# schwallergroup/matinvent

Hardware: AMD Instinct MI355X
Metric: crystal structures/sec (1000-step reverse diffusion) (higher is better)
Workload: dtype f32 via 2-plane fp16 split (3 fp16 MFMA terms, f32 accumulate)

## Files before the change

### matinvent_amd/csrc/edge_stage.hip

```cpp
#include <mutex>

#include <cstdio>
#include <cstdlib>
#include "net.h"
#include "gemm_split.h"
#define MI_LOOP_BARRIER() __builtin_amdgcn_s_barrier()
#define MI_RING_WAIT(w) asm volatile("s_waitcnt vmcnt(20)" : "+v"((w)[0][0]), "+v"((w)[0][1]), "+v"((w)[1][0]), "+v"((w)[1][1]))

namespace mi {

extern int g_edge2_train;
int g_edge2_fused = 1;

#if MI_PLANES_FP16

struct EdgeGemm2Args {
    Planes A;
    const u16* W2f;
    const float* b2;
    const float* dsc;
    const int* src;
    const int* rowptr;
    float* part;
    int E, N;
    const int* tab = nullptr;
    float* Z2 = nullptr;
    unsigned long long* clk;
};

constexpr int EG2_TAB = 2 + 128 + 128;
__global__ __launch_bounds__(128) void edge2_tables_kernel(const int* __restrict__ src, const int* __restrict__ rowptr, int E, int N, int* __restrict__ tab) {
    const int tile = blockIdx.x, tid = threadIdx.x, row0 = tile * 128;
    if (row0 >= E) return;
    const int nrows = E - row0 < 128 ? E - row0 : 128;
    const int node_first = src[row0];
    int* t = tab + (size_t)tile * EG2_TAB;
    const int r = row0 + tid, node = node_first + tid;
    t[2 + tid] = r < E ? src[r] - node_first : -1;
    t[130 + tid] = node < N ? tile - (rowptr[node] >> 7) : 0;
    if (tid == 0) {
        t[0] = node_first;
        t[1] = src[row0 + nrows - 1] - node_first + 1;
    }
}

constexpr int EG2B_STAGE = 2 * 128 * 64, EG2B_NST = 4;
constexpr int EG2B_LDS = EG2B_NST * EG2B_STAGE + 128 * 4 + 128 * 4;

template <int D, bool SAVE_Z = false>
__global__ __launch_bounds__(256) __attribute__((amdgpu_waves_per_eu(2, 2))) void edge_gemm2b_kernel(EdgeGemm2Args a) {
    constexpr int H = 512, KS = H / 16, KT = H / 32;
    extern __shared__ __attribute__((aligned(16))) unsigned char smem[];
    int* srcl = reinterpret_cast<int*>(smem + EG2B_NST * EG2B_STAGE);
    int* slotb = srcl + 128;
    const int tid = threadIdx.x, lane = tid & 63, wave = __builtin_amdgcn_readfirstlane(tid >> 6);
    const int l31 = lane & 31, kg = lane >> 5;
    const int id = blockIdx.x, slot = id >> 3, half = slot & 1, tile = (slot >> 1) * 8 + (id & 7);
    const int row0 = tile * 128;
    if (row0 >= a.E) return;
    const int nrows = a.E - row0 < 128 ? a.E - row0 : 128;
    int stamp_i = 0;
    auto stamp = [&]() {
        if (a.clk && tid == 0) a.clk[(size_t)(tile * 2 + half) * 8 + stamp_i] = __builtin_amdgcn_s_memtime();
        ++stamp_i;
    };
    stamp();
    if (a.clk && tid == 0) a.clk[(size_t)(tile * 2 + half) * 8 + 4] = __builtin_amdgcn_s_memrealtime();

    const int* tab = a.tab + (size_t)tile * EG2_TAB;
    int t_srcl = -1, t_slotb = 0;
    if (tid < 128) {
        t_srcl = tab[2 + tid];
        t_slotb = tab[130 + tid];
    }
    const int node_first = tab[0], cnt_tab = tab[1];

    const __amdgpu_buffer_rsrc_t rsa = uniform_rsrc(a.A.base + a.A.tile(tile, 0), a.A.KT * 24576);
    const int voffa = (lane >> 2) * 64 + (((lane & 3) ^ ((lane >> 4) & 3)) << 4);
    auto dma_tile = [&](int kt, int st) {
#pragma unroll
        for (int q = 0; q < 4; ++q) {
            const int piece = wave * 4 + q;
            __builtin_amdgcn_raw_ptr_buffer_load_lds(rsa, (__attribute__((address_space(3))) void*)(smem + st * EG2B_STAGE + piece * 1024), 16, voffa,
                                                     kt * 24576 + (piece >> 3) * 8192 + (piece & 7) * 1024, 0, 0);
        }
    };
    dma_tile(0, 0);
    dma_tile(1, 1);
    dma_tile(2, 2);

    int voffw[2];
#pragma unroll
    for (int t = 0; t < 2; ++t) voffw[t] = lane * 16 + ((8 * half + 2 * wave + t) * KS) * 2048;
    u32x4 ring[D][2][2];
    const u32x4 rsw_s = rsrc_words(a.W2f, H * H * 4);
    auto ring_load = [&](int ks, u32x4 (&w)[2][2]) {
        const int soff = __builtin_amdgcn_readfirstlane(ks * 2048);
#pragma unroll
        for (int t = 0; t < 2; ++t) {
            asm volatile("buffer_load_dwordx4 %0, %1, %2, %3 offen" : "=v"(w[t][0]) : "v"(voffw[t]), "s"(rsw_s), "s"(soff));
            asm volatile("buffer_load_dwordx4 %0, %1, %2, %3 offen offset:1024" : "=v"(w[t][1]) : "v"(voffw[t]), "s"(rsw_s), "s"(soff));
        }
    };
#pragma unroll
    for (int d = 0; d < D; ++d) ring_load(d, ring[d]);

    if (tid < 128) {
        srcl[tid] = t_srcl;
        slotb[tid] = t_slotb;
    }
    const float os = a.dsc[1] * (1.f / PL_SW), s_m2 = a.dsc[2], inv_m2 = a.dsc[3];

    f32x16 acc[4][2];
#pragma unroll
    for (int i = 0; i < 4; ++i)
#pragma unroll
        for (int j = 0; j < 2; ++j)
#pragma unroll
            for (int r = 0; r < 16; ++r) acc[i][j][r] = 0.f;
    const unsigned lds0 = (unsigned)(uintptr_t)(__attribute__((address_space(3))) unsigned char*)smem;
    unsigned rd_off[2];
#pragma unroll
    for (int s2 = 0; s2 < 2; ++s2) rd_off[s2] = lds0 + (unsigned)(l31 * 64 + (((2 * s2 + kg) ^ ((l31 >> 2) & 3)) * 16));
    auto read_a = [&](int st, int s2, f16x8 (&af)[4][2]) {
        const unsigned va = rd_off[s2] + (unsigned)st * EG2B_STAGE;
#define MI_RD128(dst, off) asm volatile("ds_read_b128 %0, %1 offset:%2" : "=v"(dst) : "v"(va), "n"(off))
        MI_RD128(af[0][0], 0 * 2048);        MI_RD128(af[0][1], 0 * 2048 + 8192);
        MI_RD128(af[1][0], 1 * 2048);        MI_RD128(af[1][1], 1 * 2048 + 8192);
        MI_RD128(af[2][0], 2 * 2048);        MI_RD128(af[2][1], 2 * 2048 + 8192);
        MI_RD128(af[3][0], 3 * 2048);        MI_RD128(af[3][1], 3 * 2048 + 8192);
#undef MI_RD128
    };
    auto mma = [&](const u32x4 (&w)[2][2], f16x8 (&af)[4][2]) {
#pragma unroll
        for (int ip = 0; ip < 2; ++ip) {
            if (ip == 0) asm volatile("s_waitcnt lgkmcnt(4)" : "+v"(af[0][0]), "+v"(af[0][1]), "+v"(af[1][0]), "+v"(af[1][1]));
            else asm volatile("s_waitcnt lgkmcnt(0)" : "+v"(af[2][0]), "+v"(af[2][1]), "+v"(af[3][0]), "+v"(af[3][1]));
#pragma unroll
            for (int term = MI_TERM0; term < 3; ++term)
#pragma unroll
                for (int i = 2 * ip; i < 2 * ip + 2; ++i)
#pragma unroll
                    for (int j = 0; j < 2; ++j)
                        acc[i][j] = __builtin_amdgcn_mfma_f32_32x32x16_f16(af[i][term == 0 ? 1 : 0], __builtin_bit_cast(f16x8, w[j][term == 1 ? 1 : 0]), acc[i][j], 0, 0, 0);
        }
    };
    static_assert(D == 4, "two k-tiles of ring per unrolled pair of iterations");
#pragma unroll 1
    for (int kt = 0; kt < KT; kt += 2) {
#pragma unroll
        for (int h2 = 0; h2 < 2; ++h2) {
            const int k = kt + h2;
            if (k == 0 || k >= KT - 3) asm volatile("s_waitcnt vmcnt(0)" ::: "memory");
            else asm volatile("s_waitcnt vmcnt(24)" ::: "memory");
            MI_LOOP_BARRIER();
            if (k == 0) stamp();
            if (k + 3 < KT) dma_tile(k + 3, (k + 3) & 3);
            f16x8 af[4][2];
#pragma unroll
            for (int s2 = 0; s2 < 2; ++s2) {
                read_a(k & 3, s2, af);
                MI_RING_WAIT(ring[2 * h2 + s2]);
                mma(ring[2 * h2 + s2], af);
                if (2 * k + s2 + D < KS) ring_load(2 * k + s2 + D, ring[2 * h2 + s2]);
                __builtin_amdgcn_sched_barrier(0);
            }
        }
    }
    stamp();

    if constexpr (SAVE_Z) {
        __syncthreads();
        float* stage = reinterpret_cast<float*>(smem) + wave * 1152;
#pragma unroll
        for (int i = 0; i < 4; ++i)
#pragma unroll
            for (int j = 0; j < 2; ++j) {
                const int rb = row0 + i * 32, cb = half * 256 + wave * 64 + j * 32;
#pragma unroll
                for (int r = 0; r < 16; ++r) stage[((r & 3) + 8 * (r >> 2) + 4 * kg) * 36 + l31] = acc[i][j][r] * os;
                __builtin_amdgcn_wave_barrier();
#pragma unroll
                for (int u = 0; u < 2; ++u) {
                    const int q = lane + 64 * u, rl = q >> 2, c8 = (q & 3) * 8;
                    const int row = rb + rl, col = cb + c8;
                    f32x4 z0 = *reinterpret_cast<const f32x4*>(stage + rl * 36 + c8);
                    f32x4 z1 = *reinterpret_cast<const f32x4*>(stage + rl * 36 + c8 + 4);
                    if (row < a.E) {
                        z0 += *reinterpret_cast<const f32x4*>(a.b2 + col);
                        z1 += *reinterpret_cast<const f32x4*>(a.b2 + col + 4);
                        float* d = a.Z2 + (size_t)row * H + col;
                        *reinterpret_cast<f32x4*>(d) = z0;
                        *reinterpret_cast<f32x4*>(d + 4) = z1;
                    }
                }
                __builtin_amdgcn_wave_barrier();
            }
    }

    const int cnt = nrows > 0 ? cnt_tab : 0;
    u16* sfr = reinterpret_cast<u16*>(smem);
    unsigned sat = 0;
    const int nlb = (cnt + 31) >> 5;
    __syncthreads();
    for (int f = tid; f < nlb * 8 * 64; f += 256) {
        const int ln = f & 63, fu = (f >> 6) & 1, frb = (f >> 7) & 3, fq = f >> 9;
        const int me = fq * 32 + (ln & 31), fkg = ln >> 5;
        u32x4 w;
#pragma unroll
        for (int i2 = 0; i2 < 4; ++i2) {
            const int ia = 2 * i2, ib = 2 * i2 + 1;
            const int ra = frb * 32 + 4 * fkg + 8 * (2 * fu + (ia >> 2)) + (ia & 3), rbb = frb * 32 + 4 * fkg + 8 * (2 * fu + (ib >> 2)) + (ib & 3);
            w[i2] = (srcl[ra] == me ? 0x3C00u : 0u) | (srcl[rbb] == me ? 0x3C000000u : 0u);
        }
        *reinterpret_cast<u32x4*>(sfr + (size_t)f * 8) = w;
    }
    __syncthreads();
#pragma unroll
    for (int j = 0; j < 2; ++j) {
        __builtin_amdgcn_sched_barrier(0);
        const int col = half * 256 + wave * 64 + j * 32 + l31;
        const float bcol = a.b2[col];
#pragma unroll 1
        for (int lb0 = 0; lb0 < nlb; lb0 += 2) {
            const bool two = lb0 + 1 < nlb;
            f32x16 ps[2];
#pragma unroll
            for (int q = 0; q < 2; ++q)
#pragma unroll
                for (int r = 0; r < 16; ++r) ps[q][r] = 0.f;
#pragma unroll
            for (int rb = 0; rb < 4; ++rb) {
                const f32x16 av = acc[rb][j];
#pragma unroll
                for (int u = 0; u < 2; ++u) {
                    f16x8 mh, ml;
#pragma unroll
                    for (int idx = 0; idx < 8; idx += 2) {
                        const float v0 = silu_fast(av[8 * u + idx] * os + bcol), v1 = silu_fast(av[8 * u + idx + 1] * os + bcol);
                        unsigned p[3];
                        pl_split_pair_acc(v0, v1, s_m2, p, sat);
                        const f16x2 h = __builtin_bit_cast(f16x2, p[0]), lo = __builtin_bit_cast(f16x2, p[1]);
                        mh[idx] = h[0]; mh[idx + 1] = h[1];
                        ml[idx] = lo[0]; ml[idx + 1] = lo[1];
                    }
#pragma unroll
                    for (int q = 0; q < 2; ++q) {
                        if (q == 1 && !two) break;
                        const f16x8 sf = *reinterpret_cast<const f16x8*>(sfr + (size_t)((((lb0 + q) * 4 + rb) * 2 + u) * 64 + lane) * 8);
                        ps[q] = __builtin_amdgcn_mfma_f32_32x32x16_f16(sf, ml, ps[q], 0, 0, 0);
                        ps[q] = __builtin_amdgcn_mfma_f32_32x32x16_f16(sf, mh, ps[q], 0, 0, 0);
                    }
                    __builtin_amdgcn_sched_barrier(0);
                }
            }
#pragma unroll
            for (int q = 0; q < 2; ++q)
#pragma unroll
                for (int r = 0; r < 16; ++r) {
                    const int loc = (lb0 + q) * 32 + (r & 3) + 8 * (r >> 2) + 4 * kg;
                    if (loc < cnt) a.part[((size_t)slotb[loc] * a.N + node_first + loc) * H + col] = ps[q][r] * inv_m2;
                }
        }
    }
    stamp();
    if (a.clk && tid == 0) a.clk[(size_t)(tile * 2 + half) * 8 + 5] = __builtin_amdgcn_s_memrealtime();
    sat_report(sat);
}

template <bool EXT, bool LEAN = false>
__global__ __launch_bounds__(256) __attribute__((amdgpu_waves_per_eu(2, 2))) void gemm_rt_kernel(Planes A, const u16* __restrict__ Wf, int M, int N, int K,
                                                                                                 PlanesEpilogue pe, unsigned long long* __restrict__ clk) {
    const int KS = K >> 4, KT = K >> 5;
    extern __shared__ __attribute__((aligned(16))) unsigned char smem[];
    M = pe.rows(M);
    const int tid = threadIdx.x, lane = tid & 63, wave = __builtin_amdgcn_readfirstlane(tid >> 6);
    int stamp_i = 0;
    auto stamp = [&]() {
        if (clk && tid == 0) clk[(size_t)blockIdx.x * 8 + stamp_i] = __builtin_amdgcn_s_memtime();
        ++stamp_i;
    };
    stamp();
    if (clk && tid == 0) clk[(size_t)blockIdx.x * 8 + 4] = __builtin_amdgcn_s_memrealtime();
    const int l31 = lane & 31, kg = lane >> 5;
    const int ncb = N >> 8;
    const int id = blockIdx.x, slot = id >> 3, cb = slot % ncb, tile = (slot / ncb) * 8 + (id & 7);
    const int row0 = tile * 128;
    if (row0 >= M) return;

    const __amdgpu_buffer_rsrc_t rsa = uniform_rsrc(A.base + A.tile(tile, 0), A.KT * 24576);
    const int voffa = (lane >> 2) * 64 + (((lane & 3) ^ ((lane >> 4) & 3)) << 4);
    auto dma_tile = [&](int kt, int st) {
#pragma unroll
        for (int q = 0; q < 4; ++q) {
            const int piece = wave * 4 + q;
            __builtin_amdgcn_raw_ptr_buffer_load_lds(rsa, (__attribute__((address_space(3))) void*)(smem + st * EG2B_STAGE + piece * 1024), 16, voffa,
                                                     kt * 24576 + (piece >> 3) * 8192 + (piece & 7) * 1024, 0, 0);
        }
    };
    dma_tile(0, 0);
    dma_tile(1, 1);
    dma_tile(2, 2);

    int voffw[2];
#pragma unroll
    for (int t = 0; t < 2; ++t) voffw[t] = lane * 16 + ((8 * cb + 2 * wave + t) * KS) * 2048;
    u32x4 ring[4][2][2];
    const u32x4 rsw_s = rsrc_words(Wf, N * K * 4);
    auto ring_load = [&](int ks, u32x4 (&w)[2][2]) {
        const int soff = __builtin_amdgcn_readfirstlane(ks * 2048);
#pragma unroll
        for (int t = 0; t < 2; ++t) {
            asm volatile("buffer_load_dwordx4 %0, %1, %2, %3 offen" : "=v"(w[t][0]) : "v"(voffw[t]), "s"(rsw_s), "s"(soff));
            asm volatile("buffer_load_dwordx4 %0, %1, %2, %3 offen offset:1024" : "=v"(w[t][1]) : "v"(voffw[t]), "s"(rsw_s), "s"(soff));
        }
    };
#pragma unroll
    for (int d = 0; d < 4; ++d) ring_load(d, ring[d]);

    f32x16 acc[4][2];
#pragma unroll
    for (int i = 0; i < 4; ++i)
#pragma unroll
        for (int j = 0; j < 2; ++j)
#pragma unroll
            for (int r = 0; r < 16; ++r) acc[i][j][r] = 0.f;
    const unsigned lds0 = (unsigned)(uintptr_t)(__attribute__((address_space(3))) unsigned char*)smem;
    unsigned rd_off[2];
#pragma unroll
    for (int s2 = 0; s2 < 2; ++s2) rd_off[s2] = lds0 + (unsigned)(l31 * 64 + (((2 * s2 + kg) ^ ((l31 >> 2) & 3)) * 16));
    auto read_a = [&](int st, int s2, f16x8 (&af)[4][2]) {
        const unsigned va = rd_off[s2] + (unsigned)st * EG2B_STAGE;
#define MI_RD128(dst, off) asm volatile("ds_read_b128 %0, %1 offset:%2" : "=v"(dst) : "v"(va), "n"(off))
        MI_RD128(af[0][0], 0 * 2048);        MI_RD128(af[0][1], 0 * 2048 + 8192);
        MI_RD128(af[1][0], 1 * 2048);        MI_RD128(af[1][1], 1 * 2048 + 8192);
        MI_RD128(af[2][0], 2 * 2048);        MI_RD128(af[2][1], 2 * 2048 + 8192);
        MI_RD128(af[3][0], 3 * 2048);        MI_RD128(af[3][1], 3 * 2048 + 8192);
#undef MI_RD128
    };
    auto mma = [&](const u32x4 (&w)[2][2], f16x8 (&af)[4][2]) {
#pragma unroll
        for (int ip = 0; ip < 2; ++ip) {
            if (ip == 0) asm volatile("s_waitcnt lgkmcnt(4)" : "+v"(af[0][0]), "+v"(af[0][1]), "+v"(af[1][0]), "+v"(af[1][1]));
            else asm volatile("s_waitcnt lgkmcnt(0)" : "+v"(af[2][0]), "+v"(af[2][1]), "+v"(af[3][0]), "+v"(af[3][1]));
#pragma unroll
            for (int term = MI_TERM0; term < 3; ++term)
#pragma unroll
                for (int i = 2 * ip; i < 2 * ip + 2; ++i)
#pragma unroll
                    for (int j = 0; j < 2; ++j)
// ... 441 lines not shown
```

### matinvent_amd/csrc/net.h

```cpp
#pragma once
#include <mutex>

#include "common.h"
#include "gemm.h"

struct ParamInfo {
    std::string name;
    int64_t off, numel;
    int rows, cols;
};

struct mi_net {
    mi_net_config cfg;
    int H, L, F, TD, KP, NT;
    int edge_in;
    std::vector<ParamInfo> params;
    int64_t nparams = 0;
    const float* theta = nullptr;
    uint64_t param_epoch = 0;
    float* freqs = nullptr;
    bool have_freqs = false;
    float* Whh = nullptr;
    float* Wff_p = nullptr;
    float* W2_p = nullptr;
    float* Wff = nullptr;
    int edge_mode = 1;
    unsigned short* Wffpl = nullptr;
    unsigned short* W2pl = nullptr;
    unsigned short* Wlnpl = nullptr;
    unsigned short* Waggpl = nullptr;
    unsigned short* Wn2pl = nullptr;
    unsigned short* Wffc = nullptr;
    unsigned short* Wnc = nullptr;
    float* wbounds = nullptr;
    int Kh = 0;
    unsigned short* Wffpl_pair = nullptr;
    float* C0 = nullptr;
    float* W2T = nullptr;
    unsigned short* W2Tpl = nullptr;
    unsigned short* W2Tf = nullptr;
    float* Wn2T = nullptr;
    float* Wn1T = nullptr;
    float* WhhT = nullptr;
    float* WaT = nullptr;
    unsigned short* Wbw = nullptr;
    float* WheadT = nullptr;
    bool prof = false;
    std::vector<hipEvent_t> ev;
    size_t ev_used = 0;
    hipEvent_t ev_origin = nullptr;
    std::mutex prof_mu;

    int64_t off(const std::string& name) const;
    const float* p(const std::string& name) const { return theta + off(name); }
    size_t whh_stride() const { return (size_t)2 * H * H; }
    size_t wff_stride() const { return (size_t)(KP / 4) * NT * 256; }
    size_t w2_stride() const { return (size_t)NT * NT * 4 * 256; }
};

struct Tape {
    bool allocated = false, valid = false;
    float *cat = nullptr, *Z1 = nullptr, *Z2 = nullptr, *Xpre = nullptr, *Ypre = nullptr, *lnstat = nullptr, *gf = nullptr;
    float *atom_types = nullptr, *t_emb = nullptr, *lattices = nullptr, *frac = nullptr;
    const float *in_types = nullptr, *in_temb = nullptr, *in_lat = nullptr, *in_frac = nullptr;
    bool borrow_inputs = false;
    float *dh = nullptr, *dY = nullptr, *dXa = nullptr, *Xa = nullptr, *dcat = nullptr, *dPQ = nullptr, *dG = nullptr, *dgf = nullptr,
          *dlo = nullptr, *dtproj = nullptr, *M1 = nullptr, *dM1 = nullptr, *FF = nullptr, *scratch = nullptr;
    float *nz_lat = nullptr, *nz_frac = nullptr, *nz_types = nullptr, *tar_x = nullptr, *rnd_l = nullptr, *rnd_t = nullptr, *d_l = nullptr,
          *d_x = nullptr, *d_t = nullptr, *Lb = nullptr, *KLb = nullptr;
    float* lnpart = nullptr;
    float* dsc_layers = nullptr;
    unsigned short* M1pl_l = nullptr;
    size_t m1pl_stride = 0;
    unsigned short *DmPl = nullptr, *DpPl = nullptr;
    bool dsc_layers_valid = false;
    size_t scratch_floats = 0;
    int wslots = 0, wcap = 0, wcur = 0;
    float *w_dY = nullptr, *w_Xa = nullptr, *w_dXa = nullptr, *w_cat = nullptr, *w_dPQ = nullptr;
    float *w_dlo = nullptr, *w_gf = nullptr, *w_dtype = nullptr, *w_dcoord = nullptr, *w_hf = nullptr, *w_dh = nullptr, *w_x1 = nullptr, *w_dtproj = nullptr,
          *w_temb = nullptr, *w_eXa = nullptr, *w_types = nullptr;
    bool head_window() const { return wslots > 0 && w_hf != nullptr; }
};

struct mi_batch {
    int B = 0, N = 0, H = 0, L = 0;
    int64_t E = 0;
    int64_t E_cap = 0;
    const int* e_dev = nullptr;
    int64_t e_hint = 0;
    bool knn_nosync = false;
    int nslots = 1;
    int seg_shift = 5;
    int knn = 0, max_neighbors = 0, cap_per_node = 0, deg_cap = 0, nmax = 0;
    int64_t Np = 0;
    int *pair_i = nullptr, *pair_j = nullptr, *pair_e1 = nullptr , *pair_e2 = nullptr , *pair_graph = nullptr,
        *e_diag = nullptr ;
    int* pair_off = nullptr;
    int nmax_fc = 0;
    float* fd = nullptr;
    int* inedge = nullptr;
    int *kn_ent = nullptr, *kn_acnt = nullptr, *kn_deg = nullptr, *kn_mcount = nullptr, *kn_eoff = nullptr, *kn_meta = nullptr,
        *kn_refpos = nullptr, *r_src = nullptr, *r_dst = nullptr;
    float* r_vec = nullptr;
    int64_t node_offset = 0, graph_offset = 0;
    std::vector<int> num_atoms_h, node_off_h;
    int *num_atoms = nullptr, *node_off = nullptr , *node2graph = nullptr, *src = nullptr, *dst = nullptr,
        *rowptr = nullptr , *edge_graph = nullptr ;
    float *x1_base = nullptr, *hf_base = nullptr;
    float* h = nullptr;
    float* cat = nullptr;
    float* PQ = nullptr;
    float* PQ0 = nullptr;
    bool pq0_valid = false;
    const void* reuse_net = nullptr;
    uint64_t reuse_epoch = 0;
    float* G = nullptr;
    float* part = nullptr;
    float* FFp = nullptr;
    float* FF = nullptr;
    float* M1 = nullptr;
    float* M2 = nullptr;
    unsigned short* FFpl = nullptr;
    unsigned short* M1pl = nullptr;
    unsigned short* m1_cur = nullptr;
    unsigned short* lnpl = nullptr;
    unsigned short* aggpl = nullptr;
    unsigned short* Xpl = nullptr;
    float* dsc = nullptr;
    unsigned* absmax = nullptr;
    int* e2_tab = nullptr;
    bool gram_valid = false;
    bool ff_built_once = false;
    int e2_tab_epoch = -1, graph_epoch = 0;
    unsigned* nc_flags = nullptr;
    float* X = nullptr;
    float* x1 = nullptr;
    float* tproj = nullptr;
    float* hf = nullptr;
    float* temb = nullptr;
    int* times = nullptr;
    float* pred_l = nullptr;
    float* pred_x = nullptr;
    float* pred_t = nullptr;
    float* x_mid = nullptr;
    float* lp_corr = nullptr;
    float* coef = nullptr;
    int coef_T = -1;
    std::vector<float> coef_h;
    int keep_lattice = 0, keep_coords = 0;
    mi::SplitK sk;
    hipStream_t hi_stream = nullptr;
    hipEvent_t hi_ev[2] = {nullptr, nullptr};
    Tape tape;
    uint64_t fwd_epoch = 0;
    float *tr_dl = nullptr, *tr_dx = nullptr, *tr_dt = nullptr;
    float *tr_sl = nullptr, *tr_sx = nullptr, *tr_st = nullptr;
    mi_batch* tr_partner = nullptr;
    uint64_t tr_epoch = 0, tr_partner_epoch = 0;
    float *pg_a = nullptr, *pg_x = nullptr, *pg_xm = nullptr, *pg_l = nullptr;
    float *pg_na = nullptr, *pg_nx = nullptr, *pg_nl = nullptr;
    float *pg_lp = nullptr, *pg_g = nullptr;
    int* pg_t = nullptr;
    float *kl_dl = nullptr, *kl_dt = nullptr, *kl_dxc = nullptr, *kl_dxp = nullptr;
    float* kl_val = nullptr;
    float* kl_pxc = nullptr;
    hipEvent_t ev_fork = nullptr, ev_join = nullptr;
    int* time_map = nullptr;
    int* time_map_buf = nullptr;
    int time_map_cap = 0;
    std::vector<int> time_map_h;
    bool cond_on = false;
    bool cond_any = false;
    int cond_levels = 0;
    int cond_table_cap = 0;
    int *cond_kt = nullptr, *cond_kx = nullptr, *cond_kl = nullptr, *cond_types0 = nullptr;
    float *cond_frac0 = nullptr, *cond_lat0 = nullptr, *cond_table = nullptr;
    std::vector<void*> allocs;
};

namespace mi {
int net_forward(mi_net* net, mi_batch* b, const float* t_emb, const float* atom_types, const float* frac,
                const float* lattices, float* lattice_out, float* coord_out, float* type_out, hipStream_t s, bool train = false,
                bool reuse_embedding = false, bool coords_only = false);
int net_tape_prepare(mi_net* net, mi_batch* b);
int net_pack_transposes(mi_net* net, hipStream_t s);
int net_backward(mi_net* net, mi_batch* b, const float* d_lat, const float* d_coord, const float* d_type, float* grad, hipStream_t s);
int net_wgrad_window(mi_net* net, mi_batch* b, int slots);
int net_wgrad_flush(mi_net* net, mi_batch* b, float* grad, hipStream_t s);
template <typename T>
int dev_alloc(mi_batch* b, T** p, size_t n);
int knn_alloc(mi_batch* b, int max_neighbors, int cap_per_node);
extern int g_node_bwd, g_node_bwd_min_blocks;
size_t node_bwd_pack_elems(int H);
bool node_bwd_supported(const mi_net* net, const mi_batch* b);
int node_bwd_pack(mi_net* net, int l, const float* W1, const float* Wn0, const float* Wn2, hipStream_t s);
int node_bwd(mi_net* net, mi_batch* b, int l, const float* dPQ, float* dh, float* dY, float* dXa, float* Xa, float* lnpart, unsigned* dcat_absmax, hipStream_t s);
bool node_chain_supported(const mi_net* net);
size_t node_chain_pack_elems(int H);
int node_chain_pack(mi_net* net, int l, const float* W1, const float* Wn0, const float* Wn2, const float* W2, hipStream_t s);
bool edge_gemm1_supported(const mi_net* net, int64_t M);
int edge_gemm1_pack(mi_net* net, int l, const float* W1, hipStream_t s);
bool edge_gemm2_supported(const mi_net* net);
extern int g_edge2_train;
extern int g_node_train;
extern int g_node_cols;
extern int g_ablate_skip;
int edge_gemm2(mi_net* net, mi_batch* b, int layer, hipStream_t s, float* Z2 = nullptr);
int node_chain(mi_net* net, mi_batch* b, int l, hipStream_t s, bool train = false);
int time_embedding_mapped(const mi_batch* b, const int* steps, int k_all, const float* freqs, int B, int TD, float* out, hipStream_t s);
int time_map_check(const mi_batch* b, int T, const char* what);
int time_map_same(const mi_batch* p, const mi_batch* q, const char* what);
int condition_check(const mi_batch* b, int T, const char* what);
int condition_impose(const mi_batch* b, int level, uint64_t seed, float* atom_types, float* frac, float* lattices, float* rec_types, float* rec_frac,
                     float* rec_lat, hipStream_t s);
extern int g_knn_nosync;
int knn_build(mi_batch* b, const float* frac, const float* lattices, hipStream_t s, bool nosync = false);
}
```

### matinvent_amd/csrc/node_chain.hip

```cpp
#include <mutex>

#include "net.h"
#include "gemm_split.h"

namespace mi {

unsigned long long* g_node_clk = nullptr;
int g_node_fused = 1;
int g_node_split = 1;
int g_node_split_max_blocks = 256;
int g_ablate_skip = 0;
int g_node_touch_min_blocks = 64;
int g_node_cols = 3;
int g_node_cols_auto_blocks = 36;
int g_node_cols_b_max = 0;
int g_node_cols_fused_max = 256;

#if MI_PLANES_FP16

__global__ void pack_frag_kernel(const float* __restrict__ W, int ld, int rows, int K, u16* __restrict__ dst, int row0) {
    const int KS = K / 16;
    const int64_t idx = (int64_t)blockIdx.x * blockDim.x + threadIdx.x;
    if (idx >= (int64_t)rows * (K / 8)) return;
    const int r = (int)(idx / (K / 8)), ch = (int)(idx % (K / 8));
    const int R = row0 + r, ct = R >> 5, l31 = R & 31, ks = ch >> 1, kg = ch & 1;
    u32x4 pk[2];
#pragma unroll
    for (int i = 0; i < 4; ++i) {
        unsigned p[3];
        pl_split_pair(W[(size_t)r * ld + ch * 8 + 2 * i], W[(size_t)r * ld + ch * 8 + 2 * i + 1], PL_SW, p);
        pk[0][i] = p[0];
        pk[1][i] = p[1];
    }
#pragma unroll
    for (int pl = 0; pl < 2; ++pl)
        *reinterpret_cast<u32x4*>(dst + ((((size_t)ct * KS + ks) * 2 + pl) * 64 + kg * 32 + l31) * 8) = pk[pl];
}

struct NodeChainArgs {
    int N = 0;
    const float* part = nullptr;
    const int* rowptr = nullptr;
    int seg_shift = 5;
    const unsigned* slotmask = nullptr;
    int nslots = 0;
    const float* xpart = nullptr;
    int ld_xpart = 0;
    const u16* Wagg = nullptr;
    const u16* Wn2 = nullptr;
    const float* b0 = nullptr;
    const float* b2 = nullptr;
    const float* dsc = nullptr;
    const float* h_in = nullptr;
    float* h_out = nullptr;
    const float* ln_w = nullptr;
    const float* ln_b = nullptr;
    float* hf = nullptr;
    const u16* Wln = nullptr;
    float* PQ = nullptr;
    unsigned* absmax = nullptr;
    unsigned long long* clk = nullptr;
    float* t_agg = nullptr;
    int ld_agg = 0;
    float* t_xpre = nullptr;
    float* t_ypre = nullptr;
    float* t_ln = nullptr;
    int ld_ln = 0;
    float* t_lnstat = nullptr;
    int a_only = 0, split_b = 0;
    int touch = 0;
    int stages = 0, gy = 1, npad = 0;
    u16* xpl = nullptr;
    unsigned* flags = nullptr;
};

template <int H>
struct NodeChainCfg {
    static constexpr int KS = H / 16, ROWB = 2 * H + 16, PLB = 32 * ROWB, HLD = H + 4;
    static constexpr int LDS = 2 * PLB + 32 * HLD * 4;
};

template <int H, int NW, int D, bool PQ = true>
__global__ __launch_bounds__(64 * NW) __attribute__((amdgpu_waves_per_eu(NW / 4, NW / 4))) void node_chain_kernel(NodeChainArgs a) {
    using C = NodeChainCfg<H>;
    constexpr int KS = C::KS, ROWB = C::ROWB, PLB = C::PLB, HLD = C::HLD, CW = H / NW, TW = CW / 32, RPW = 32 / NW;
    static_assert(KS % D == 0 && KS >= 2 * D && CW % 32 == 0, "ring depth / column split");
    extern __shared__ __attribute__((aligned(16))) unsigned char smem[];
    unsigned char* P = smem;
    float* Hs = reinterpret_cast<float*>(smem + 2 * PLB);
    const int tid = threadIdx.x, lane = tid & 63, wave = __builtin_amdgcn_readfirstlane(tid >> 6);
    const int l31 = lane & 31, kg = lane >> 5;
    const int row0 = blockIdx.x * 32, N = a.N;

    int stamp_i = 0;
    auto stamp = [&]() {
        if (a.clk && tid == 0) a.clk[(size_t)blockIdx.x * 16 + stamp_i] = __builtin_amdgcn_s_memtime();
        ++stamp_i;
    };
    stamp();
    float touch_dummy = 0.f;
    if (a.touch) {
        const int bl = (int)(blockIdx.x + gridDim.x * blockIdx.y), nb = (int)(gridDim.x * gridDim.y);
        const int part = bl >> 3, nparts = (nb - (bl & 7) + 7) >> 3;
        auto touch = [&](const void* base, int bytes) {
            const int nlines = bytes >> 7;
            for (int l0 = part * (64 * NW); l0 < nlines; l0 += nparts * (64 * NW)) {
                const int line = l0 + tid;
                if (line < nlines) asm volatile("global_load_dword %0, %1, off" : "+v"(touch_dummy) : "v"(reinterpret_cast<const char*>(base) + (size_t)line * 128));
            }
        };
        const int wbytes = H * H * 4;
        if (a.part != nullptr) {
            touch(a.Wagg, wbytes);
            touch(a.Wn2, wbytes);
        }
        if (a.Wln != nullptr && !a.a_only) touch(a.Wln + (size_t)(a.split_b ? blockIdx.y : 0) * H * H * 2, (a.split_b ? 1 : 3) * wbytes);
    }
    u32x4 ring[D][TW][2];
    f32x16 acc[TW];
    int voff[TW];
#pragma unroll
    for (int t = 0; t < TW; ++t) voff[t] = lane * 16 + t * KS * 2048;
    auto ring_load = [&](const __amdgpu_buffer_rsrc_t& rs, int ct0, int ks, u32x4 (&w)[TW][2]) {
        const int so = (ct0 * KS + ks) * 2048;
#pragma unroll
        for (int t = 0; t < TW; ++t)
#pragma unroll
            for (int pl = 0; pl < 2; ++pl) w[t][pl] = __builtin_amdgcn_raw_buffer_load_b128(rs, voff[t] + pl * 1024, so, 0);
    };
    auto ring_fill = [&](const __amdgpu_buffer_rsrc_t& rs, int ct0) {
#pragma unroll
        for (int d = 0; d < D; ++d) ring_load(rs, ct0, d, ring[d]);
    };
    auto read_act = [&](int ks, f16x8 (&af)[2]) {
#pragma unroll
        for (int pl = 0; pl < 2; ++pl) af[pl] = *reinterpret_cast<const f16x8*>(P + pl * PLB + l31 * ROWB + (2 * ks + kg) * 16);
    };
    auto mma_step = [&](auto tr, const u32x4 (&w)[TW][2], const f16x8 (&af)[2]) {
        constexpr bool TR = decltype(tr)::value;
#pragma unroll
        for (int term = MI_TERM0; term < 3; ++term)
#pragma unroll
            for (int t = 0; t < TW; ++t) {
                const f16x8 wv = __builtin_bit_cast(f16x8, w[t][term == 1 ? 1 : 0]);
                const f16x8 av = af[term == 0 ? 1 : 0];
                if constexpr (TR) acc[t] = __builtin_amdgcn_mfma_f32_32x32x16_f16(wv, av, acc[t], 0, 0, 0);
                else acc[t] = __builtin_amdgcn_mfma_f32_32x32x16_f16(av, wv, acc[t], 0, 0, 0);
            }
    };
    auto run = [&](auto tr, const __amdgpu_buffer_rsrc_t& rs, int ct0) {
#pragma unroll
        for (int t = 0; t < TW; ++t)
#pragma unroll
            for (int r = 0; r < 16; ++r) acc[t][r] = 0.f;
        f16x8 af[2][2];
        read_act(0, af[0]);
#pragma unroll 1
        for (int ks0 = 0; ks0 < KS - D; ks0 += D) {
#pragma unroll
            for (int d = 0; d < D; ++d) {
                read_act(ks0 + d + 1, af[(d + 1) & 1]);
                mma_step(tr, ring[d], af[d & 1]);
                ring_load(rs, ct0, ks0 + d + D, ring[d]);
                __builtin_amdgcn_sched_barrier(0);
            }
        }
#pragma unroll
        for (int d = 0; d < D; ++d) {
            if (d + 1 < D) read_act(KS - D + d + 1, af[(d + 1) & 1]);
            mma_step(tr, ring[d], af[d & 1]);
        }
    };
    using TRt = std::true_type;
    using TRf = std::false_type;
    static_assert(D % 2 == 0, "the activation fragments alternate between two register sets");

    const bool phaseA = a.part != nullptr, phaseB = a.Wln != nullptr;
    const int wsz = H * H * 4;
    if (phaseA) {
        const __amdgpu_buffer_rsrc_t rs_agg = uniform_rsrc(a.Wagg, wsz);
        const float s_agg = a.dsc[2];
        unsigned sat = 0;
        {
            const int c0 = lane * 8;
            const bool act = c0 < H;
            int e0[RPW], e1[RPW];
            int rp;
            {
                const int idx = row0 + wave * RPW + lane;
                rp = a.rowptr[idx < N ? idx : N];
            }
#pragma unroll
            for (int r = 0; r < RPW; ++r) {
                const int i = row0 + wave * RPW + r;
                e0[r] = i < N ? __builtin_amdgcn_readlane(rp, r) : 0;
                e1[r] = i < N ? __builtin_amdgcn_readlane(rp, r + 1) : 0;
            }
            f32x4 xsum[RPW], ysum[RPW];
            bool any[RPW];
            if (a.slotmask) {
                unsigned mk[RPW];
#pragma unroll
                for (int r = 0; r < RPW; ++r) {
                    const int i = row0 + wave * RPW + r;
                    mk[r] = i < N ? a.slotmask[i] : 0u;
                    xsum[r] = ysum[r] = f32x4{0.f, 0.f, 0.f, 0.f};
                    any[r] = mk[r] != 0u && e1[r] > e0[r];
                }
                for (int sl = 0; sl < a.nslots; ++sl) {
#pragma unroll
                    for (int r = 0; r < RPW; ++r) {
                        const int i = row0 + wave * RPW + r;
                        if (act && ((mk[r] >> sl) & 1u)) {
                            const float* p = a.part + ((size_t)sl * N + i) * H + c0;
                            xsum[r] += *reinterpret_cast<const f32x4*>(p);
                            ysum[r] += *reinterpret_cast<const f32x4*>(p + 4);
                        }
                    }
                }
                ring_fill(rs_agg, wave * TW);
            } else {
            f32x4 x[RPW], y[RPW], x1[RPW], y1[RPW];
#pragma unroll
            for (int r = 0; r < RPW; ++r) {
                const int i = row0 + wave * RPW + r;
                const int ns = e1[r] > e0[r] ? ((e1[r] - 1) >> a.seg_shift) - (e0[r] >> a.seg_shift) + 1 : 0;
                x[r] = y[r] = x1[r] = y1[r] = f32x4{0.f, 0.f, 0.f, 0.f};
                if (act && ns > 0) {
                    const float* p = a.part + (size_t)i * H + c0;
                    x[r] = *reinterpret_cast<const f32x4*>(p);
                    y[r] = *reinterpret_cast<const f32x4*>(p + 4);
                    if (ns > 1) {
                        x1[r] = *reinterpret_cast<const f32x4*>(p + (size_t)N * H);
                        y1[r] = *reinterpret_cast<const f32x4*>(p + (size_t)N * H + 4);
                    }
                }
            }
            ring_fill(rs_agg, wave * TW);
#pragma unroll
            for (int r = 0; r < RPW; ++r) {
                const int i = row0 + wave * RPW + r;
                const int ns = e1[r] > e0[r] ? ((e1[r] - 1) >> a.seg_shift) - (e0[r] >> a.seg_shift) + 1 : 0;
                f32x4 xs = x[r], ys = y[r];
                if (act && ns > 1) {
                    xs += x1[r];
                    ys += y1[r];
                    for (int sl = 2; sl < ns; ++sl) {
                        const float* p = a.part + ((size_t)sl * N + i) * H + c0;
                        xs += *reinterpret_cast<const f32x4*>(p);
                        ys += *reinterpret_cast<const f32x4*>(p + 4);
                    }
                }
                xsum[r] = xs;
                ysum[r] = ys;
                any[r] = ns > 0;
            }
            }
#pragma unroll
            for (int r = 0; r < RPW; ++r) {
                const int row = wave * RPW + r;
                if (!act) continue;
                f32x4 xs = xsum[r], ys = ysum[r];
                if (any[r]) {
                    const float d = (float)(e1[r] - e0[r]);
#pragma unroll
                    for (int k = 0; k < 4; ++k) {
                        xs[k] = xs[k] / d;
                        ys[k] = ys[k] / d;
                    }
                }
                if (a.t_agg && row0 + row < N) {
                    float* o = a.t_agg + (size_t)(row0 + row) * a.ld_agg + c0;
                    *reinterpret_cast<f32x4*>(o) = xs;
                    *reinterpret_cast<f32x4*>(o + 4) = ys;
                }
                u32x4 pk[2];
                unsigned pr[3];
                pl_split_pair_acc(xs[0], xs[1], s_agg, pr, sat); pk[0][0] = pr[0]; pk[1][0] = pr[1];
                pl_split_pair_acc(xs[2], xs[3], s_agg, pr, sat); pk[0][1] = pr[0]; pk[1][1] = pr[1];
                pl_split_pair_acc(ys[0], ys[1], s_agg, pr, sat); pk[0][2] = pr[0]; pk[1][2] = pr[1];
                pl_split_pair_acc(ys[2], ys[3], s_agg, pr, sat); pk[0][3] = pr[0]; pk[1][3] = pr[1];
#pragma unroll
                for (int pl = 0; pl < 2; ++pl) *reinterpret_cast<u32x4*>(P + pl * PLB + row * ROWB + c0 * 2) = pk[pl];
            }
        }
        __syncthreads();
        stamp();
        f32x4 xq[TW][4];
        auto load_xq = [&]() {
            const int i = row0 + l31;
            const int ic = i < N ? i : N - 1;
#pragma unroll
            for (int t = 0; t < TW; ++t)
#pragma unroll
                for (int q = 0; q < 4; ++q) {
                    xq[t][q] = *reinterpret_cast<const f32x4*>(a.xpart + (size_t)ic * a.ld_xpart + wave * CW + t * 32 + 8 * q + 4 * kg);
                }
        };
        if constexpr (PQ) load_xq();
        run(TRt{}, rs_agg, wave * TW);
        stamp();
        if constexpr (!PQ) load_xq();
        const __amdgpu_buffer_rsrc_t rs_n2 = uniform_rsrc(a.Wn2, wsz);
        f32x4 hq[TW][4];
        auto load_hq = [&]() {
            const int i = row0 + l31;
            const int ic = i < N ? i : N - 1;
#pragma unroll
            for (int t = 0; t < TW; ++t)
#pragma unroll
                for (int q = 0; q < 4; ++q) {
                    hq[t][q] = *reinterpret_cast<const f32x4*>(a.h_in + (size_t)ic * H + wave * CW + t * 32 + 8 * q + 4 * kg);
                }
        };
        if constexpr (PQ) load_hq();
        __syncthreads();
        {
            const float os = a.dsc[3] * (1.f / PL_SW), s_x = a.dsc[4];
            const int i = row0 + l31;
            f32x4 bq[TW][4];
#pragma unroll
            for (int t = 0; t < TW; ++t)
#pragma unroll
                for (int q = 0; q < 4; ++q) bq[t][q] = *reinterpret_cast<const f32x4*>(a.b0 + wave * CW + t * 32 + 8 * q + 4 * kg);
            ring_fill(rs_n2, wave * TW);
#pragma unroll
            for (int t = 0; t < TW; ++t)
#pragma unroll
                for (int q = 0; q < 4; ++q) {
                    const int c4 = wave * CW + t * 32 + 8 * q + 4 * kg;
                    float v[4];
                    f32x4 zpre;
#pragma unroll
                    for (int k = 0; k < 4; ++k) zpre[k] = (acc[t][4 * q + k] * os + bq[t][q][k]) + xq[t][q][k];
                    if (a.t_xpre && i < N) *reinterpret_cast<f32x4*>(a.t_xpre + (size_t)i * H + c4) = zpre;
#pragma unroll
                    for (int k = 0; k < 4; ++k) v[k] = i < N ? silu_fast(zpre[k]) : 0.f;
                    unsigned p01[3], p23[3];
                    pl_split_pair_acc(v[0], v[1], s_x, p01, sat);
                    pl_split_pair_acc(v[2], v[3], s_x, p23, sat);
#pragma unroll
                    for (int pl = 0; pl < 2; ++pl) {
                        const uint2 wv = make_uint2(p01[pl], p23[pl]);
                        *reinterpret_cast<uint2*>(P + pl * PLB + l31 * ROWB + c4 * 2) = wv;
                    }
                }
            sat_report(sat);
        }
        __syncthreads();
        stamp();
        run(TRt{}, rs_n2, wave * TW);
        stamp();
        if constexpr (!PQ) load_hq();
        {
            const float os = a.dsc[5] * (1.f / PL_SW);
            const int i = row0 + l31;
            f32x4 bq[TW][4];
#pragma unroll
            for (int t = 0; t < TW; ++t)
#pragma unroll
                for (int q = 0; q < 4; ++q) bq[t][q] = *reinterpret_cast<const f32x4*>(a.b2 + wave * CW + t * 32 + 8 * q + 4 * kg);
            if (phaseB) ring_fill(uniform_rsrc(a.Wln, 3 * wsz), wave * TW);
#pragma unroll
            for (int t = 0; t < TW; ++t)
#pragma unroll
                for (int q = 0; q < 4; ++q) {
                    const int c4 = wave * CW + t * 32 + 8 * q + 4 * kg;
                    f32x4 o, ypre;
#pragma unroll
                    for (int k = 0; k < 4; ++k) ypre[k] = acc[t][4 * q + k] * os + bq[t][q][k];
                    if (a.t_ypre && i < N) *reinterpret_cast<f32x4*>(a.t_ypre + (size_t)i * H + c4) = ypre;
#pragma unroll
                    for (int k = 0; k < 4; ++k) o[k] = silu_fast(ypre[k]) + hq[t][q][k];
                    *reinterpret_cast<f32x4*>(Hs + l31 * HLD + c4) = o;
                }
        }
        __syncthreads();
        stamp();
    } else if (phaseB) {
        ring_fill(uniform_rsrc(a.Wln, 3 * wsz), ((a.split_b ? (int)blockIdx.y : 0) * H + wave * CW) / 32);
    }
    if (a.touch) asm volatile("s_waitcnt vmcnt(0)" : "+v"(touch_dummy));
    if (a.a_only) {
        const int c0 = lane * 8;
        if (c0 < H)
#pragma unroll 2
            for (int r = 0; r < RPW; ++r) {
                const int row = wave * RPW + r, i = row0 + row;
                if (i < N) {
                    *reinterpret_cast<f32x4*>(a.h_out + (size_t)i * H + c0) = *reinterpret_cast<const f32x4*>(Hs + row * HLD + c0);
                    *reinterpret_cast<f32x4*>(a.h_out + (size_t)i * H + c0 + 4) = *reinterpret_cast<const f32x4*>(Hs + row * HLD + c0 + 4);
                }
            }
        return;
    }
    const int pass_lo = a.split_b ? (int)blockIdx.y : 0, pass_hi = a.split_b ? (int)blockIdx.y + 1 : 3;
    const bool tape_w = !a.split_b || blockIdx.y == 0;
    unsigned sat_ln = 0;
    {
        const int c0 = lane * 8;
        const bool act = c0 < H;
        f32x4 w0 = {0.f, 0.f, 0.f, 0.f}, w1 = w0, b0 = w0, b1 = w0;
        if (act) {
            w0 = *reinterpret_cast<const f32x4*>(a.ln_w + c0);
            w1 = *reinterpret_cast<const f32x4*>(a.ln_w + c0 + 4);
            b0 = *reinterpret_cast<const f32x4*>(a.ln_b + c0);
            b1 = *reinterpret_cast<const f32x4*>(a.ln_b + c0 + 4);
        }
#pragma unroll 2
        for (int r = 0; r < RPW; ++r) {
            const int row = wave * RPW + r, i = row0 + row;
            f32x4 x = {0.f, 0.f, 0.f, 0.f}, y = {0.f, 0.f, 0.f, 0.f};
            if (act && i < N) {
                if (phaseA) {
                    x = *reinterpret_cast<const f32x4*>(Hs + row * HLD + c0);
                    y = *reinterpret_cast<const f32x4*>(Hs + row * HLD + c0 + 4);
                    *reinterpret_cast<f32x4*>(a.h_out + (size_t)i * H + c0) = x;
                    *reinterpret_cast<f32x4*>(a.h_out + (size_t)i * H + c0 + 4) = y;
                } else {
                    x = *reinterpret_cast<const f32x4*>(a.h_in + (size_t)i * H + c0);
                    y = *reinterpret_cast<const f32x4*>(a.h_in + (size_t)i * H + c0 + 4);
                }
            }
            const float mean = wave_sum(((x[0] + x[1]) + (x[2] + x[3])) + ((y[0] + y[1]) + (y[2] + y[3]))) / (float)H;
            float q = 0.f;
            if (act) {
#pragma unroll
                for (int k = 0; k < 4; ++k) {
                    const float da = x[k] - mean, db = y[k] - mean;
                    q += da * da + db * db;
                }
            }
            const float var = wave_sum(q) / (float)H;
            const float rstd = 1.0f / sqrtf(var + 1e-5f);
            f32x4 o0 = {0.f, 0.f, 0.f, 0.f}, o1 = o0;
            if (act && i < N) {
#pragma unroll
                for (int k = 0; k < 4; ++k) {
                    o0[k] = (x[k] - mean) * rstd * w0[k] + b0[k];
                    o1[k] = (y[k] - mean) * rstd * w1[k] + b1[k];
                }
                if (a.hf) {
                    *reinterpret_cast<f32x4*>(a.hf + (size_t)i * H + c0) = o0;
                    *reinterpret_cast<f32x4*>(a.hf + (size_t)i * H + c0 + 4) = o1;
                }
                if (a.t_ln && tape_w) {
                    *reinterpret_cast<f32x4*>(a.t_ln + (size_t)i * a.ld_ln + c0) = o0;
                    *reinterpret_cast<f32x4*>(a.t_ln + (size_t)i * a.ld_ln + c0 + 4) = o1;
                }
            }
            if (a.t_lnstat && tape_w && lane == 0 && i < N) {
                a.t_lnstat[2 * (size_t)i] = mean;
                a.t_lnstat[2 * (size_t)i + 1] = rstd;
            }
            if (act && phaseB) {
                u32x4 pk[2];
                unsigned pr[3];
                pl_split_pair_acc(o0[0], o0[1], PL_S_LN, pr, sat_ln); pk[0][0] = pr[0]; pk[1][0] = pr[1];
                pl_split_pair_acc(o0[2], o0[3], PL_S_LN, pr, sat_ln); pk[0][1] = pr[0]; pk[1][1] = pr[1];
                pl_split_pair_acc(o1[0], o1[1], PL_S_LN, pr, sat_ln); pk[0][2] = pr[0]; pk[1][2] = pr[1];
                pl_split_pair_acc(o1[2], o1[3], PL_S_LN, pr, sat_ln); pk[0][3] = pr[0]; pk[1][3] = pr[1];
#pragma unroll
                for (int pl = 0; pl < 2; ++pl) *reinterpret_cast<u32x4*>(P + pl * PLB + row * ROWB + c0 * 2) = pk[pl];
            }
        }
    }
    sat_report(sat_ln);
    if (!phaseB) return;
    __syncthreads();
    stamp();
    {
        const __amdgpu_buffer_rsrc_t rs_ln = uniform_rsrc(a.Wln, 3 * wsz);
        constexpr float os = 1.f / (PL_S_LN * PL_SW);
        float m = 0.f;
#pragma unroll 1
        for (int pass = pass_lo; pass < pass_hi; ++pass) {
            const int ct0 = (pass * H + wave * CW) / 32;
            run(TRf{}, rs_ln, ct0);
            stamp();
            if (pass + 1 < pass_hi) ring_fill(rs_ln, ((pass + 1) * H + wave * CW) / 32);
#pragma unroll
            for (int t = 0; t < TW; ++t) {
                const int col = pass * H + wave * CW + t * 32 + l31;
#pragma unroll
                for (int r = 0; r < 16; ++r) {
                    const int i = row0 + (r & 3) + 8 * (r >> 2) + 4 * kg;
                    const float v = acc[t][r] * os;
                    if (i < N) {
                        a.PQ[(size_t)i * (3 * H) + col] = v;
                        m = fmaxf(m, fabsf(v));
                    }
                }
            }
        }
        if (a.absmax) {
#pragma unroll
            for (int o = 32; o > 0; o >>= 1) m = fmaxf(m, __shfl_xor(m, o, 64));
            if (lane == 0) atomicMax(a.absmax, __float_as_uint(m));
        }
        stamp();
    }
}

template <int H, int NW, int D, bool PQ = true>
static int node_chain_launch(const NodeChainArgs& a, hipStream_t s) {
    static std::once_flag once;
    static hipError_t attr_err = hipSuccess;
    std::call_once(once, [] { attr_err = hipFuncSetAttribute((const void*)node_chain_kernel<H, NW, D, PQ>, hipFuncAttributeMaxDynamicSharedMemorySize, NodeChainCfg<H>::LDS); });
    MI_HIP(attr_err);
    hipLaunchKernelGGL((node_chain_kernel<H, NW, D, PQ>), dim3(cdiv(a.N, 32), a.split_b ? 3 : 1), dim3(64 * NW), NodeChainCfg<H>::LDS, s, a);
    MI_KERNEL_CHECK();
    return MI_OK;
}


template <int H>
struct NodeColsCfg {
    static constexpr int KS = H / 16, ROWB = 2 * H + 16, PLB = 32 * ROWB, NCG = H / 128;
    static constexpr int LDS = 2 * PLB + 32;
};

template <int H, int D, int ST>
__global__ __launch_bounds__(256) __attribute__((amdgpu_waves_per_eu(2, 2))) void node_cols_kernel(NodeChainArgs a) {
    using C = NodeColsCfg<H>;
    constexpr int KS = C::KS, ROWB = C::ROWB, PLB = C::PLB, NCG = C::NCG, RPW = 8;
    static_assert(KS % D == 0 && KS >= 2 * D && D % 2 == 0 && H % 128 == 0, "ring depth / column groups");
    extern __shared__ __attribute__((aligned(16))) unsigned char smem[];
    unsigned char* P = smem;
    const int tid = threadIdx.x, lane = tid & 63, wave = __builtin_amdgcn_readfirstlane(tid >> 6);
    const int l31 = lane & 31, kg = lane >> 5;
    const int N = a.N, nblk = (N + 31) >> 5, gy = a.gy;
    const int bid = blockIdx.x, xcd = bid & 7, j = bid >> 3;
    const int cgw = j % gy, rb = (j / gy) * 8 + xcd;
    if (rb >= nblk) return;
    const int row0 = rb * 32;

    int stamp_i = 0;
    auto stamp = [&]() {
        if (a.clk && tid == 0) a.clk[(size_t)bid * 16 + stamp_i] = __builtin_amdgcn_s_memtime();
        ++stamp_i;
    };
    stamp();
    u32x4 ring[D][2];
    f32x16 acc;
    const int voff = lane * 16;
    auto tile_rsrc = [&](const u16* W, int ct) { return uniform_rsrc(W + (size_t)ct * KS * 1024, KS * 2048); };
    auto ring_load = [&](const __amdgpu_buffer_rsrc_t& rs, int vo, int d, u32x4 (&w)[2]) {
#pragma unroll
        for (int pl = 0; pl < 2; ++pl) w[pl] = __builtin_amdgcn_raw_buffer_load_b128(rs, vo + pl * 1024, d * 2048, 0);
    };
    auto ring_fill = [&](const __amdgpu_buffer_rsrc_t& rs) {
#pragma unroll
        for (int d = 0; d < D; ++d) ring_load(rs, voff, d, ring[d]);
    };
    auto read_act = [&](int ks, f16x8 (&af)[2]) {
#pragma unroll
        for (int pl = 0; pl < 2; ++pl) af[pl] = *reinterpret_cast<const f16x8*>(P + pl * PLB + l31 * ROWB + (2 * ks + kg) * 16);
    };
    auto mma_step = [&](auto tr, const u32x4 (&w)[2], const f16x8 (&af)[2]) {
        constexpr bool TR = decltype(tr)::value;
#pragma unroll
        for (int term = MI_TERM0; term < 3; ++term) {
            const f16x8 wv = __builtin_bit_cast(f16x8, w[term == 1 ? 1 : 0]);
            const f16x8 av = af[term == 0 ? 1 : 0];
            if constexpr (TR) acc = __builtin_amdgcn_mfma_f32_32x32x16_f16(wv, av, acc, 0, 0, 0);
            else acc = __builtin_amdgcn_mfma_f32_32x32x16_f16(av, wv, acc, 0, 0, 0);
        }
    };
    auto run = [&](auto tr, const __amdgpu_buffer_rsrc_t& rs) {
#pragma unroll
        for (int r = 0; r < 16; ++r) acc[r] = 0.f;
        f16x8 af[2][2];
        read_act(0, af[0]);
#pragma unroll 1
        for (int ks0 = 0; ks0 < KS; ks0 += D) {
            const int vo = voff + (ks0 + D) * 2048;
#pragma unroll
            for (int d = 0; d < D; ++d) {
                read_act(ks0 + d + 1, af[(d + 1) & 1]);
                mma_step(tr, ring[d], af[d & 1]);
                ring_load(rs, vo, d, ring[d]);
                __builtin_amdgcn_sched_barrier(0);
            }
        }
    };
    using TRt = std::true_type;
    using TRf = std::false_type;
    auto handover = [&](int seam) {
        __syncthreads();
        if (tid == 0) {
            __builtin_amdgcn_fence(__ATOMIC_RELEASE, "agent");
            asm volatile("s_waitcnt vmcnt(0)" ::: "memory");
            unsigned* f = a.flags + 2 * rb + seam;
            __hip_atomic_fetch_add(f, 1u, __ATOMIC_RELAXED, __HIP_MEMORY_SCOPE_AGENT);
            while (__hip_atomic_load(f, __ATOMIC_RELAXED, __HIP_MEMORY_SCOPE_AGENT) < (unsigned)gy) __builtin_amdgcn_s_sleep(1);
            __builtin_amdgcn_fence(__ATOMIC_ACQUIRE, "agent");
        }
        __syncthreads();
    };

    const int cg = cgw;
    const int ct_a = cg * 4 + wave;
    const int ccol = cg * 128 + wave * 32;
    if constexpr ((ST & 1) != 0) {
        const __amdgpu_buffer_rsrc_t rs_agg = tile_rsrc(a.Wagg, ct_a);
        const float s_agg = a.dsc[2];
        unsigned sat = 0;
        {
            const int c0 = lane * 8;
            const bool act = c0 < H;
            int rp;
            {
                const int idx = row0 + wave * RPW + lane;
                rp = a.rowptr[idx < N ? idx : N];
            }
#pragma unroll 1
            for (int half = 0; half < 2; ++half) {
                constexpr int RH = RPW / 2;
                int e0[RH], e1[RH];
#pragma unroll
                for (int r = 0; r < RH; ++r) {
                    const int i = row0 + wave * RPW + half * RH + r;
                    e0[r] = i < N ? __builtin_amdgcn_readlane(rp, half * RH + r) : 0;
                    e1[r] = i < N ? __builtin_amdgcn_readlane(rp, half * RH + r + 1) : 0;
                }
                f32x4 x[RH], y[RH], x1[RH], y1[RH];
#pragma unroll
                for (int r = 0; r < RH; ++r) {
                    const int i = row0 + wave * RPW + half * RH + r;
                    const int ns = e1[r] > e0[r] ? ((e1[r] - 1) >> a.seg_shift) - (e0[r] >> a.seg_shift) + 1 : 0;
                    x[r] = y[r] = x1[r] = y1[r] = f32x4{0.f, 0.f, 0.f, 0.f};
                    if (act && ns > 0) {
                        const float* p = a.part + (size_t)i * H + c0;
                        x[r] = *reinterpret_cast<const f32x4*>(p);
                        y[r] = *reinterpret_cast<const f32x4*>(p + 4);
                        if (ns > 1) {
                            x1[r] = *reinterpret_cast<const f32x4*>(p + (size_t)N * H);
                            y1[r] = *reinterpret_cast<const f32x4*>(p + (size_t)N * H + 4);
                        }
                    }
                }
                if (half == 1) ring_fill(rs_agg);
#pragma unroll
                for (int r = 0; r < RH; ++r) {
                    const int row = wave * RPW + half * RH + r, i = row0 + row;
                    const int ns = e1[r] > e0[r] ? ((e1[r] - 1) >> a.seg_shift) - (e0[r] >> a.seg_shift) + 1 : 0;
                    f32x4 xs = x[r], ys = y[r];
                    if (act && ns > 1) {
                        xs += x1[r];
                        ys += y1[r];
                        for (int sl = 2; sl < ns; ++sl) {
                            const float* p = a.part + ((size_t)sl * N + i) * H + c0;
                            xs += *reinterpret_cast<const f32x4*>(p);
                            ys += *reinterpret_cast<const f32x4*>(p + 4);
                        }
                    }
                    if (!act) continue;
                    if (ns > 0) {
                        const float d = (float)(e1[r] - e0[r]);
#pragma unroll
                        for (int k = 0; k < 4; ++k) {
                            xs[k] = xs[k] / d;
                            ys[k] = ys[k] / d;
                        }
                    }
                    if (a.t_agg && cgw == 0 && i < N) {
                        float* o = a.t_agg + (size_t)i * a.ld_agg + c0;
                        *reinterpret_cast<f32x4*>(o) = xs;
                        *reinterpret_cast<f32x4*>(o + 4) = ys;
                    }
                    u32x4 pk[2];
                    unsigned pr[3];
                    pl_split_pair_acc(xs[0], xs[1], s_agg, pr, sat); pk[0][0] = pr[0]; pk[1][0] = pr[1];
                    pl_split_pair_acc(xs[2], xs[3], s_agg, pr, sat); pk[0][1] = pr[0]; pk[1][1] = pr[1];
                    pl_split_pair_acc(ys[0], ys[1], s_agg, pr, sat); pk[0][2] = pr[0]; pk[1][2] = pr[1];
                    pl_split_pair_acc(ys[2], ys[3], s_agg, pr, sat); pk[0][3] = pr[0]; pk[1][3] = pr[1];
#pragma unroll
                    for (int pl = 0; pl < 2; ++pl) *reinterpret_cast<u32x4*>(P + pl * PLB + row * ROWB + c0 * 2) = pk[pl];
                }
            }
        }
        __syncthreads();
        stamp();
        f32x4 xq[4];
        {
            const int i = row0 + l31;
            const int ic = i < N ? i : N - 1;
#pragma unroll
            for (int q = 0; q < 4; ++q) {
                xq[q] = *reinterpret_cast<const f32x4*>(a.xpart + (size_t)ic * a.ld_xpart + ccol + 8 * q + 4 * kg);
            }
        }
        run(TRt{}, rs_agg);
        stamp();
        {
            const float os = a.dsc[3] * (1.f / PL_SW), s_x = a.dsc[4];
            const int i = row0 + l31;
            f32x4 bq[4];
#pragma unroll
            for (int q = 0; q < 4; ++q) bq[q] = *reinterpret_cast<const f32x4*>(a.b0 + ccol + 8 * q + 4 * kg);
#pragma unroll
            for (int q = 0; q < 4; ++q) {
                const int c4 = ccol + 8 * q + 4 * kg;
                float v[4];
                f32x4 zpre;
#pragma unroll
                for (int k = 0; k < 4; ++k) zpre[k] = (acc[4 * q + k] * os + bq[q][k]) + xq[q][k];
                if (a.t_xpre && i < N) *reinterpret_cast<f32x4*>(a.t_xpre + (size_t)i * H + c4) = zpre;
#pragma unroll
                for (int k = 0; k < 4; ++k) v[k] = i < N ? silu_fast(zpre[k]) : 0.f;
                unsigned p01[3], p23[3];
                pl_split_pair_acc(v[0], v[1], s_x, p01, sat);
                pl_split_pair_acc(v[2], v[3], s_x, p23, sat);
#pragma unroll
                for (int pl = 0; pl < 2; ++pl)
                    *reinterpret_cast<uint2*>(a.xpl + ((size_t)pl * a.npad + i) * H + c4) = make_uint2(p01[pl], p23[pl]);
            }
            sat_report(sat);
        }
        stamp();
        if constexpr ((ST & 2) != 0) handover(0);
    }
    if constexpr ((ST & 2) != 0) {
        const __amdgpu_buffer_rsrc_t rs_n2 = tile_rsrc(a.Wn2, ct_a);
        {
            constexpr int PPR = H / 8, NP = 32 * PPR / 256;
// ... 380 lines not shown
```

Before: 55.31.

## Overlay node-chain h' rows onto activation planes to shrink LDS footprint

The node-chain kernel's h' staging buffer now aliases the two fp16 activation planes instead of sitting after them, which cuts the kernel's LDS request. The aim is for a node-chain workgroup and an edge-GEMM workgroup to fit on one CU together, as the new static_assert checks. To keep the aliasing safe, a barrier is added before the epilogue writes h', and the LayerNorm pass now loads all rows into registers and then hits a barrier before later phases overwrite the planes. The cost is extra barriers and more register pressure from fully unrolled per-row buffers.

```diff
diff --git a/matinvent_amd/csrc/edge_stage.hip b/matinvent_amd/csrc/edge_stage.hip
--- a/matinvent_amd/csrc/edge_stage.hip
+++ b/matinvent_amd/csrc/edge_stage.hip
@@ -46,6 +46,7 @@
 
 constexpr int EG2B_STAGE = 2 * 128 * 64, EG2B_NST = 4;
 constexpr int EG2B_LDS = EG2B_NST * EG2B_STAGE + 128 * 4 + 128 * 4;
+static_assert(NodeChainCfg<512>::LDS + EG2B_LDS <= 160 * 1024, "node chain + one edge-GEMM workgroup per CU");
 
 template <int D, bool SAVE_Z = false>
 __global__ __launch_bounds__(256) __attribute__((amdgpu_waves_per_eu(2, 2))) void edge_gemm2b_kernel(EdgeGemm2Args a) {
diff --git a/matinvent_amd/csrc/net.h b/matinvent_amd/csrc/net.h
--- a/matinvent_amd/csrc/net.h
+++ b/matinvent_amd/csrc/net.h
@@ -198,6 +198,12 @@
 bool node_chain_supported(const mi_net* net);
 size_t node_chain_pack_elems(int H);
 int node_chain_pack(mi_net* net, int l, const float* W1, const float* Wn0, const float* Wn2, const float* W2, hipStream_t s);
+template <int H>
+struct NodeChainCfg {
+    static constexpr int KS = H / 16, ROWB = 2 * H + 16, PLB = 32 * ROWB, HLD = H + 4;
+    static constexpr int LDS = 2 * PLB;
+    static_assert(32 * HLD * 4 <= LDS, "the h' rows overlay the two activation planes");
+};
 bool edge_gemm1_supported(const mi_net* net, int64_t M);
 int edge_gemm1_pack(mi_net* net, int l, const float* W1, hipStream_t s);
 bool edge_gemm2_supported(const mi_net* net);
diff --git a/matinvent_amd/csrc/node_chain.hip b/matinvent_amd/csrc/node_chain.hip
--- a/matinvent_amd/csrc/node_chain.hip
+++ b/matinvent_amd/csrc/node_chain.hip
@@ -74,11 +74,6 @@
     unsigned* flags = nullptr;
 };
 
-template <int H>
-struct NodeChainCfg {
-    static constexpr int KS = H / 16, ROWB = 2 * H + 16, PLB = 32 * ROWB, HLD = H + 4;
-    static constexpr int LDS = 2 * PLB + 32 * HLD * 4;
-};
 
 template <int H, int NW, int D, bool PQ = true>
 __global__ __launch_bounds__(64 * NW) __attribute__((amdgpu_waves_per_eu(NW / 4, NW / 4))) void node_chain_kernel(NodeChainArgs a) {
@@ -87,7 +82,7 @@
     static_assert(KS % D == 0 && KS >= 2 * D && CW % 32 == 0, "ring depth / column split");
     extern __shared__ __attribute__((aligned(16))) unsigned char smem[];
     unsigned char* P = smem;
-    float* Hs = reinterpret_cast<float*>(smem + 2 * PLB);
+    float* Hs = reinterpret_cast<float*>(smem);
     const int tid = threadIdx.x, lane = tid & 63, wave = __builtin_amdgcn_readfirstlane(tid >> 6);
     const int l31 = lane & 31, kg = lane >> 5;
     const int row0 = blockIdx.x * 32, N = a.N;
@@ -351,6 +346,7 @@
         stamp();
         run(TRt{}, rs_n2, wave * TW);
         stamp();
+        __syncthreads();
         if constexpr (!PQ) load_hq();
         {
             const float os = a.dsc[5] * (1.f / PL_SW);
@@ -407,21 +403,32 @@
             b0 = *reinterpret_cast<const f32x4*>(a.ln_b + c0);
             b1 = *reinterpret_cast<const f32x4*>(a.ln_b + c0 + 4);
         }
-#pragma unroll 2
+        f32x4 hx[RPW], hy[RPW];
+#pragma unroll
         for (int r = 0; r < RPW; ++r) {
             const int row = wave * RPW + r, i = row0 + row;
-            f32x4 x = {0.f, 0.f, 0.f, 0.f}, y = {0.f, 0.f, 0.f, 0.f};
+            hx[r] = hy[r] = f32x4{0.f, 0.f, 0.f, 0.f};
             if (act && i < N) {
                 if (phaseA) {
-                    x = *reinterpret_cast<const f32x4*>(Hs + row * HLD + c0);
-                    y = *reinterpret_cast<const f32x4*>(Hs + row * HLD + c0 + 4);
-                    *reinterpret_cast<f32x4*>(a.h_out + (size_t)i * H + c0) = x;
-                    *reinterpret_cast<f32x4*>(a.h_out + (size_t)i * H + c0 + 4) = y;
+                    hx[r] = *reinterpret_cast<const f32x4*>(Hs + row * HLD + c0);
+                    hy[r] = *reinterpret_cast<const f32x4*>(Hs + row * HLD + c0 + 4);
+                    *reinterpret_cast<f32x4*>(a.h_out + (size_t)i * H + c0) = hx[r];
+                    *reinterpret_cast<f32x4*>(a.h_out + (size_t)i * H + c0 + 4) = hy[r];
                 } else {
-                    x = *reinterpret_cast<const f32x4*>(a.h_in + (size_t)i * H + c0);
-                    y = *reinterpret_cast<const f32x4*>(a.h_in + (size_t)i * H + c0 + 4);
-                }
-            }
+                    hx[r] = *reinterpret_cast<const f32x4*>(a.h_in + (size_t)i * H + c0);
+                    hy[r] = *reinterpret_cast<const f32x4*>(a.h_in + (size_t)i * H + c0 + 4);
+                }
+            }
+        }
+        if (phaseA && phaseB) {
+            asm volatile("s_waitcnt lgkmcnt(0)" ::: "memory");
+            __builtin_amdgcn_s_barrier();
+            asm volatile("" ::: "memory");
+        }
+#pragma unroll
+        for (int r = 0; r < RPW; ++r) {
+            const int row = wave * RPW + r, i = row0 + row;
+            const f32x4 x = hx[r], y = hy[r];
             const float mean = wave_sum(((x[0] + x[1]) + (x[2] + x[3])) + ((y[0] + y[1]) + (y[2] + y[3]))) / (float)H;
             float q = 0.f;
             if (act) {
```

Measured after the change: 55.27, median of 2. About the same (-0.1%).
